# dylanpeifer/deepgroebner

Measured on AMD Instinct MI355X. Metric: env steps/sec (polynomial additions) on 3-20-10-weighted, batch=4096, 1/2/4/8 GPU, higher is better.
Workload: dtype u16 exponents / u32 GF(32003)

## Files before the change

deepgroebner_amd/csrc/bbx_common.h:

```cpp
#pragma once
#include <stdbool.h>
#include <stddef.h>
#include <stdint.h>

#define BBX_P 32003u
#define BBX_POLICY_MAX_ROWS 2048
#define BBX_MAXVARS 8
#ifdef __HIPCC__
#define BBX_HD __host__ __device__
#else
#define BBX_HD
#endif

enum {
  BBX_ST_OK = 0,
  BBX_ST_G_FULL = 1,
  BBX_ST_P_FULL = 2,
  BBX_ST_ARENA_FULL = 3,
  BBX_ST_POLY_TOO_LONG = 4,
  BBX_ST_DEG_OVERFLOW = 5,
  BBX_ST_STARVED = 6,
  BBX_ST_BAD_ACTION = 7,
  BBX_ST_RUNAWAY = 9,
  BBX_ST_GEN_FAIL = 10,
// ... 204 lines not shown
  bool dev = false;
  int at = 0;
  auto uniform = [&](uint32_t scaling, uint32_t past, uint32_t magic) {
    uint32_t ret = acc.raw(at++) - 1u;
    if (ret >= past) { dev = true; ret = 0; }
    return bbx_gen_div(ret, scaling, magic);
  };
  auto degree = [&]() {
    const uint32_t r1 = acc.raw(at), r2 = acc.raw(at + 1);
    at += 2;
    const double pr = bbx_gen_canonical(r1, r2);
    int d = 0;
    for (int i = 0; i < ncp; i++) d += acc.cp(i) < pr ? 1 : 0;
    return d;
  };
  r.c = (flags & 2u) ? BBX_P - 1u : 1u + uniform(67104u, 2147462208u, 64004u);
  int d1 = 0, d2 = 0;
  if (ncp != 0) {
    d1 = degree();
    d2 = (flags & 1u) ? d1 : degree();
  }
  const BbxGenRow row1 = acc.row(d1), row2 = acc.row(d2);
  const uint32_t j1 = row1.off + uniform(row1.scaling, row1.past, row1.magic);
  const uint32_t j2 = row2.off + uniform(row2.scaling, row2.past, row2.magic);
  uint32_t m1[2], m2[2];
  acc.mono(j1, m1); acc.mono(j2, m2);
  const uint64_t k1 = (((uint64_t)m1[1] << 32) | m1[0]) ^ 0x0000FFFFFFFFFFFFull;
  const uint64_t k2 = (((uint64_t)m2[1] << 32) | m2[0]) ^ 0x0000FFFFFFFFFFFFull;
  const bool second = k2 > k1;
  r.lead[0] = second ? m2[0] : m1[0]; r.lead[1] = second ? m2[1] : m1[1];
  r.tail[0] = second ? m1[0] : m2[0]; r.tail[1] = second ? m1[1] : m2[1];
  r.deviated = dev || k1 == k2;
  return r;
}
#endif

static inline BBX_HD uint32_t bbx_coef_mulmod(uint32_t a, uint32_t b) {
  const uint32_t x = a * b;
  const uint32_t q = (uint32_t)(((uint64_t)x * 1099408559ull) >> 45);
  return x - q * BBX_P;
}
static inline BBX_HD uint32_t bbx_ginfo_hot(uint32_t rec_x, uint32_t inv) {
  const uint32_t mt = bbx_coef_mulmod(rec_x >> 16, inv);
  return mt | ((mt ? BBX_P - mt : 0u) << 16);
}
static inline BBX_HD uint32_t bbx_ginfo_record(uint32_t hot_x, uint32_t kept) { (void)hot_x; return kept; }

#define BBX_PEEL_NO_KEY 0xFFFFFFFFu
static inline BBX_HD uint32_t bbx_peel_key(uint32_t deg, uint32_t index) { return (deg << 8) | index; }
static inline BBX_HD uint32_t bbx_peel_key_deg(uint32_t key) { return key >> 8; }
static inline BBX_HD int bbx_peel_key_lane(uint32_t key) { return (int)(key & 63u); }
static inline BBX_HD int bbx_peel_key_bank(uint32_t key) { return (int)((key >> 6) & 3u); }

static inline BBX_HD uint64_t bbx_mix64(uint64_t idx, uint32_t word) {
  uint64_t z = ((idx << 32) | (uint64_t)word) + 0x9E3779B97F4A7C15ull;
  z = (z ^ (z >> 30)) * 0xBF58476D1CE4E5B9ull;
  z = (z ^ (z >> 27)) * 0x94D049BB133111EBull;
  return z ^ (z >> 31);
}
static inline BBX_HD uint32_t bbx_agent_hash32(uint32_t seed, uint32_t t) {
  return (uint32_t)(bbx_mix64((uint64_t)seed, t) >> 32);
}
static inline BBX_HD uint32_t bbx_agent_action32(uint32_t seed, uint32_t t, uint32_t rows) {
  return (uint32_t)(((uint64_t)bbx_agent_hash32(seed, t) * rows) >> 32);
}
```

deepgroebner_amd/csrc/bbx_fast.h:

```cpp
#pragma once

typedef Mono<2> M2;
template <int NBK> struct FLay {
  static constexpr int G = 64 * NBK, P = 2 * G, OVF = G > 128 ? G - 128 : 0;
  static constexpr int OFF_LM = 0, OFF_TM = 8 * G, OFF_GI = 16 * G, OFF_PR = 24 * G, OFF_SX = 24 * G + 4 * P, OFF_GC = OFF_SX + 2 * OVF;
  static constexpr int BYTES = OFF_GC + 4 * G;
};
constexpr int FNBK_WIDE = 4, FNBK_POL = 2;
static_assert(FLay<FNBK_WIDE>::BYTES == 9472 && FLay<FNBK_POL>::BYTES == 4608, "FLay: bytes per environment (DESIGN.md 4.1, LDS budget)");
static_assert(FLay<FNBK_WIDE>::OFF_GC % 4 == 0 && FLay<FNBK_WIDE>::BYTES % 16 == 0 && FLay<FNBK_POL>::BYTES % 16 == 0, "FLay: alignment of gc[] and of the next wave's region");
static_assert(16 * FLay<FNBK_WIDE>::BYTES == 151552 && 16 * FLay<FNBK_WIDE>::BYTES <= 160 * 1024, "16 environments per CU no longer fit its LDS");
static_assert(16 * (FLay<FNBK_POL>::BYTES + 4 * FLay<FNBK_POL>::P) + 66576 == 156688 && 156688 <= 160 * 1024, "policy2<128,128>: 16 environments per CU no longer fit its LDS");
constexpr uint32_t FSENT = 0xFFFFFFFFu;

struct BbxFastParams {
  char* recs; const uint32_t* qwords; const int32_t* qtail; const uint16_t* inv_table;
  const int32_t* actions; double* rewards; uint8_t* dones; int32_t* rows; int32_t* obs; BbxTraceRec* trace;
  uint32_t rec_bytes, hbmG;
  uint32_t q_env_stride, q_slot_words, q_nslots, q_fixed;
  int32_t B, nsteps, obs_rows, trace_stride, k, nvars, lim_G, lim_P;
  int32_t agent, auto_reset, set_budget, pass, obs_every_step, obs_fill, rewards_mode;
  int32_t* lite;
  int32_t done_seq;
  const uint32_t* gen;
// ... 142 lines not shown
  int budget_in = uni(ghdr->budget), rollout_pos = uni(ghdr->rollout_pos), done_in = uni(ghdr->done_last);
  if (status == BBX_ST_STARVED || status == BBX_ST_SPILL || status == BBX_ST_TIMESLICE) status = BBX_ST_OK;
  if (p.set_budget) { budget_in = bbx_st_capacity(status) ? budget_in + p.nsteps : p.nsteps; rollout_pos = 0; done_in = 0; }
  if (p.sess_target) budget_in = p.sess_target - uni(ghdr->sess_done);
  const uint32_t t_begin = PERSIST ? (uint32_t)__builtin_amdgcn_s_memrealtime() : 0u;
  int mb_action = -1;
  bool mb_pending = false;
  int pol_t0 = 0;
  if (POL > 0 && PERSIST) { int vz_; asm volatile("v_mov_b32 %0, 0" : "=v"(vz_)); pol_t0 = vz_ + (t_agent - (p.set_budget ? 0 : uni(ghdr->sess_done))); }
  if (p.pass == 1 && !(status == BBX_ST_OK && (need_reset || (budget_in > 0 && nP > 0)))) return;
  if constexpr (PERSIST) {
    if (p.sess_target && !p.set_budget && !p.mbox && uni(ghdr->status) == BBX_ST_OK && !need_reset && budget_in <= 0 &&
        nG <= (p.lim_G < FG ? p.lim_G : FG) && nP <= (p.lim_P < FP ? p.lim_P : FP)) {
      const unsigned long long w = __hip_atomic_load(p.ctl, __ATOMIC_RELAXED, __HIP_MEMORY_SCOPE_AGENT);
      if (uni((int)(uint32_t)w) <= uni(ghdr->sess_done) && (uni((int)(uint32_t)(w >> 32)) & 1)) {
        if (lane == 0) {
          const int done_last = done_in ? 1 : 0;
          const int trunc_all = ghdr->obs_trunc | ((POL == 0 && p.obs && nP > p.obs_rows) ? 1 : 0);
          ghdr->arena_used = 0; ghdr->steps_done = 0; ghdr->budget = budget_in; ghdr->done_last = done_last; ghdr->obs_trunc = trunc_all;
          if (p.dones) p.dones[env] = (uint8_t)bbx_done_flag(done_last, nP, 0);
          if (p.rows) p.rows[env] = nP;
          if (p.lite) {
            int32_t* lw = p.lite + 4 * (size_t)env;
            const int word0 = bbx_lite_word0(BBX_ST_OK, trunc_all, p.done_seq);
            if (p.done_seq) {
              lw[1] = q_head; lw[2] = budget_in; lw[3] = nP;
              __threadfence_system();
              __hip_atomic_store(lw, word0, __ATOMIC_RELEASE, __HIP_MEMORY_SCOPE_SYSTEM);
            } else *(int4*)lw = make_int4(word0, q_head, budget_in, nP);
          }
        }
        return;
      }
    }
  }
  int t_stop = t_agent + budget_in, t_event = t_agent;

#define F_HBM_PTRS(PP) \
  const uint32_t HG = (PP)->hbmG; char* grec_ = (PP)->recs + (size_t)env * (PP)->rec_bytes; \
  M2* g_lm = (M2*)(grec_ + 128);            M2* g_tm = (M2*)(grec_ + 128 + 8 * HG); \
  M2* g_slm = (M2*)(grec_ + 128 + 16 * HG); M2* g_stm = (M2*)(grec_ + 128 + 24 * HG); \
  uint2* g_gi = (uint2*)(grec_ + 128 + 40 * HG); uint2* g_si = (uint2*)(grec_ + 128 + 48 * HG); \
  uint32_t* g_pr = (uint32_t*)(grec_ + 128 + 56 * HG);
  char* lbase = smem + wave_in_block * (FLDS_BYTES + (POL > 0 ? 4 * FP : 0));
  M2* lm = (M2*)(lbase + FOFF_LM); M2* tm = (M2*)(lbase + FOFF_TM);
  uint2* gi = (uint2*)(lbase + FOFF_GI); uint32_t* pairs = (uint32_t*)(lbase + FOFF_PR);
  uint32_t* gc = (uint32_t*)(lbase + LY::OFF_GC);
  const int limG = p.lim_G < FG ? p.lim_G : FG, limP = p.lim_P < FP ? p.lim_P : FP;

  uint16_t* sx = (uint16_t*)(lbase + LY::OFF_SX);
  FastState S;
  auto clear_reducers = [&]() { f_banks<FRB>([&](auto b_) { constexpr int b = decltype(b_)::value; S.slm[b].w[0] = S.slm[b].w[1] = FSENT; }); };
  clear_reducers();
  f_banks<FRB>([&](auto b_) { constexpr int b = decltype(b_)::value; S.stm[b] = m_zero<2>(); S.sin[b] = make_uint2(0, 0); });
  bool staged_in = false;
  const bool idle0 = !PERSIST && !need_reset && nP == 0;
  if (status == BBX_ST_OK && !idle0) {
    if (nG > limG || nP > limP) status = BBX_ST_SPILL;
    else {
      F_HBM_PTRS(&p)
      f_banks<NBK>([&](auto b_) {
        constexpr int b = decltype(b_)::value;
        const int i = lane + 64 * b;
        if (i < nG) {
          if constexpr (b < FRB) { S.slm[b] = g_slm[i]; S.stm[b] = g_stm[i]; S.sin[b] = g_si[i]; }
          else sx[i - 64 * FRB] = (uint16_t)(g_si[i].y >> 16);
          const uint2 rg = g_gi[i];
          lm[i] = g_lm[i]; tm[i] = g_tm[i]; gc[i] = rg.x; gi[i] = make_uint2(bbx_ginfo_hot(rg.x, rg.y & 0xffffu), rg.y);
        }
      });
      for (int i = lane; i < nP; i += WAVE) pairs[i] = g_pr[i];
      staged_in = true;
      wave_sync();
    }
  }
  f_loads_landed();
  uint32_t PA = pairs[lane];

  uint32_t hv = bbx_agent_hash32(agent_seed, (uint32_t)((t_agent & ~63) + lane));
  int vzero; asm volatile("v_mov_b32 %0, 0" : "=v"(vzero));
  int adds = vzero, episodes = vzero, zero_red = vzero;
  int trace_pos = rollout_pos;
  long long bytes_total = 0;
  int last_nred = vzero - 1;
  int obs_rows_max = vzero;
  int t_done = vzero + (done_in ? t_agent : t_agent - 1);
  const int t_entry = vzero + t_agent;
  int t_ep0 = 0, t_lim = 0;
  if constexpr (!NOLIM) {
    t_ep0 = vzero + (t_agent - uni(ghdr->episode_steps));
    t_lim = uni(bbx_episode_tlim(t_agent - uni(ghdr->episode_steps), t_agent, p.episode_limit));
  }
  const bool tracing = TRACE && p.trace != nullptr;
  const int n = HL ? 3 : p.nvars, kk = HL ? 2 : p.k;
  const int agent = HL ? BBX_AGENT_HASH : p.agent;
  const bool auto_reset = HL ? true : p.auto_reset != 0;
  const bool obs_fill = HL ? false : p.obs_fill != 0;
  int filled_to = (!HL && p.obs_fill == 2 && p.rows) ? uni(p.rows[env]) : 0x7fffffff;
  const bool obs_step = HL ? true : (POL > 0 ? false : (p.obs_every_step && p.obs));
  const int per_row = 2 * kk;
  const int obs_row_bytes = 4 * per_row * n;
  const int o_rl = lane / per_row, o_slot = lane - o_rl * per_row;
  const int rows_per_sweep = per_row <= WAVE ? WAVE / per_row : 0;

  struct __attribute__((aligned(4))) ObsI3 { int32_t a, b, c; };
  const bool obs32 = HL ? true : (n == 3 && kk == 2 && p.obs != nullptr);
  const int o3_row = lane >> 2, o3_hi = (lane >> 1) & 1;
  const char* o3_mono = lbase + ((lane & 1) ? FOFF_TM : FOFF_LM);
  int32_t* const o3_base = obs32 ? p.obs + (size_t)env * p.obs_rows * 12 : nullptr;
  typedef int32_t ObsV3 __attribute__((ext_vector_type(3)));
  size_t o3_toff = 0;
  auto note_rows = [&]() { obs_rows_max = obs_rows_max > nP ? obs_rows_max : nP; };
  auto write_obs32 = [&]() {
    const int rows = nP < p.obs_rows ? nP : p.obs_rows;
    int32_t* ob = o3_base + o3_toff;
    asm volatile("" : "+s"(ob));
    const __amdgpu_buffer_rsrc_t rs = __builtin_amdgcn_make_buffer_rsrc((void*)ob, 0, rows * 48, 0x00020000);
    int r0 = 0;
// ... 118 lines not shown
            if (valid[b]) { eq[b] = ballot64(f_u64(L[b]) == ls) & valid[b]; dv[b] = ballot64(m_divides(Ls, L[b])); }
            bad |= eq[b] & cp[b];
          }
        });
        if (bad == 0) f_banks<BK>([&](auto b_) { constexpr int b = decltype(b_)::value; if (BK == 1 || sb == b) emit[b] |= 1ull << s; });
        f_banks<BK>([&](auto b_) { constexpr int b = decltype(b_)::value; cand[b] &= ~dv[b]; });
      }
    }
    auto stays = [&](uint32_t pr, const M2& li, const M2& lj, int k) {
      const uint32_t a0 = pk_max(li.w[0], lj.w[0]), a1 = pk_max(li.w[1], lj.w[1]);
      const uint32_t b0 = pk_max(li.w[0], f.w[0]), b1 = pk_max(li.w[1], f.w[1]);
      const uint32_t c0 = pk_max(lj.w[0], f.w[0]), c1 = pk_max(lj.w[1], f.w[1]);
      const bool fdiv = (pk_subsat(f.w[0], a0) | (pk_subsat(f.w[1], a1) & 0xffffu)) == 0;
      const bool eqi = ((a0 ^ b0) | ((a1 ^ b1) & 0xffffu)) == 0;
      const bool eqj = ((a0 ^ c0) | ((a1 ^ c1) & 0xffffu)) == 0;
      return (k < nP_old) & (k != skip) & !(fdiv & !eqi & !eqj);
    };
    const bool keep_first = stays(pr_first, li_first, lj_first, lane);
    const uint64_t mask_first = ballot64(keep_first);
    if (keep_first) pairs[f_prefix(mask_first)] = pr_first;
    int w = __popcll(mask_first);
    for (int base = WAVE; base < nP_old; base += WAVE) {
      const int k = base + lane;
      const uint32_t pr = k < nP_old ? pairs[k] : 0u;
      const bool keep = stays(pr, lm[pr & 0xffffu], lm[pr >> 16], k);
      const uint64_t mask = ballot64(keep);
      if (keep) pairs[w + f_prefix(mask)] = pr;
      w += __popcll(mask);
    }
    nP = w;
    f_banks<BK>([&](auto b_) {
      constexpr int b = decltype(b_)::value;
      if (b == 0 || emit[b]) {
        if (f_lane_in(emit[b])) pairs[nP + f_prefix(emit[b])] = (uint32_t)(lane + 64 * b) | ((uint32_t)g << 16);
        nP += __popcll(emit[b]);
      }
    });
    {
      constexpr int RB = BK < FRB ? BK : FRB;
      int pos = __popcll(ballot64(!m_gt(S.slm[0], f)));
      f_banks<RB>([&](auto b_) {
        constexpr int b = decltype(b_)::value;
        if constexpr (b > 0) if (g >= 64 * b) pos += __popcll(ballot64(!m_gt(S.slm[b], f)));
      });
      const int novf = (OVF && BK > FRB && g > 64 * FRB) ? g - 64 * FRB : 0;
      if (OVF && BK > FRB) for (int k0 = 0; k0 < novf; k0 += WAVE) {
        const int k = k0 + lane;
        const bool le = k < novf && !m_gt(lm[sx[k < novf ? k : 0]], f);
        pos += __popcll(ballot64(le));
      }
      const uint32_t inv = (uint32_t)uni((int)inv_raw);
      const uint32_t rec_x = t0.c | (t1.c << 16), hot_x = bbx_ginfo_hot(rec_x, inv);
      if (lane == 0) { lm[g] = f; tm[g] = tail; gi[g] = make_uint2(hot_x, inv | ((uint32_t)sugar << 16)); gc[g] = rec_x; }
      const uint2 ns = make_uint2(t1.c | (hot_x & 0xffff0000u), (uint32_t)sugar | ((uint32_t)g << 16));
      int ovq = -1; uint32_t ovg = 0;
      if (OVF && BK > FRB && g >= 64 * FRB) {
        if (pos >= 64 * FRB) { ovq = pos - 64 * FRB; ovg = (uint32_t)g; }
        else { ovq = 0; ovg = f_readlane(S.sin[FRB - 1].y, 63) >> 16; }
      }
      if (!(OVF && BK > FRB) || pos < 64 * FRB) {
        const int pb = RB == 1 ? 0 : pos >> 6, q = RB == 1 ? pos : pos & 63;
        uint32_t c0 = 0, c1 = 0, c2 = 0, c3 = 0, c4 = 0, c5 = 0;
        const uint32_t nv[6] = {f.w[0], f.w[1], tail.w[0], tail.w[1], ns.x, ns.y};
        f_banks<RB>([&](auto b_) {
          constexpr int b = decltype(b_)::value;
          if (RB == 1 || pb == b) {
            if constexpr (b + 1 < RB) {
              c0 = f_readlane(S.slm[b].w[0], 63); c1 = f_readlane(S.slm[b].w[1], 63); c2 = f_readlane(S.stm[b].w[0], 63);
              c3 = f_readlane(S.stm[b].w[1], 63); c4 = f_readlane(S.sin[b].x, 63); c5 = f_readlane(S.sin[b].y, 63);
            }
            f_insert6(S.slm[b].w[0], S.slm[b].w[1], S.stm[b].w[0], S.stm[b].w[1], S.sin[b].x, S.sin[b].y, nv, q);
          } else if (b > 0 && pb < b && g >= 64 * b) {
            c0 = f_shift_in(S.slm[b].w[0], c0, lane); c1 = f_shift_in(S.slm[b].w[1], c1, lane);
            c2 = f_shift_in(S.stm[b].w[0], c2, lane); c3 = f_shift_in(S.stm[b].w[1], c3, lane);
            c4 = f_shift_in(S.sin[b].x, c4, lane); c5 = f_shift_in(S.sin[b].y, c5, lane);
          }
        });
      }
      if (OVF && BK > FRB && ovq >= 0) {
        for (int k0 = ((novf - 1 - ovq) / WAVE) * WAVE; k0 >= 0; k0 -= WAVE) {
          const int k = ovq + k0 + lane;
          uint16_t v = 0;
          if (k < novf) v = sx[k];
          wave_sync();
          if (k < novf) sx[k + 1] = v;
          wave_sync();
        }
        if (lane == 0) sx[ovq] = (uint16_t)ovg;
      }
    }
    nG = g + 1;
    wave_sync();
    PA = pairs[lane];
  };

  auto install_ideal = [&](int n, bool in_order) {
    int ln = lane; asm volatile("" : "+v"(ln));
    const bool mine = ln < n;
    const M2 L = lm[ln];
    {
      const M2 T = tm[ln];
      const uint32_t cx = gi[ln].x, sugar = m_deg(L);
      if (mine) gc[ln] = 1u | (cx << 16);
      const int rk = in_order ? ln : gen_sorted_rank<2>(L, n);
      const int to = 4 * (mine ? rk : ln);
      auto put = [&](uint32_t v) { return (uint32_t)__builtin_amdgcn_ds_permute(to, (int)v); };
      S.slm[0].w[0] = put(mine ? L.w[0] : FSENT); S.slm[0].w[1] = put(mine ? L.w[1] : FSENT);
      S.stm[0].w[0] = put(T.w[0]); S.stm[0].w[1] = put(T.w[1]);
      S.sin[0].x = put(cx); S.sin[0].y = put(sugar | ((uint32_t)ln << 16));
    }
    int j = 0;
#pragma unroll
    for (int t = 1; t <= 10; t++) j += ln >= t * (t - 1) / 2 ? 1 : 0;
    const int i = ln - ((j * (j - 1)) >> 1);
    auto get = [&](int from, const M2& v) { M2 r; r.w[0] = (uint32_t)__builtin_amdgcn_ds_bpermute(4 * from, (int)v.w[0]);
                                            r.w[1] = (uint32_t)__builtin_amdgcn_ds_bpermute(4 * from, (int)v.w[1]); return r; };
    const M2 Li = get(i, L), Lj = get(j, L), Lij = m_lcm(Li, Lj);
    bool keep = ln < ((n * (n - 1)) >> 1);
    for (int k = 0; k < n; k++) {
      const M2 Lk = f_readlane(L, k);
      const M2 Lkj = m_lcm(Lk, Lj);
      const bool eq = m_eq(Lkj, Lij);
      const bool not_new = (m_divides(Lkj, Lij) && !eq) || (eq && (k < i || m_coprime(Lk, Lj)));
      const bool dropped = m_divides(Lk, Lij) && !eq && !m_eq(Lij, m_lcm(Li, Lk));
      keep = keep && !(k < j ? not_new : (k > j && dropped));
    }
    const uint64_t kept = ballot64(keep);
    if (keep) pairs[f_prefix(kept)] = (uint32_t)i | ((uint32_t)j << 16);
    nG = n; nP = __popcll(kept);
    wave_sync();
    PA = pairs[lane];
  };

#ifndef BBX_PRIO_SHIFT
#define BBX_PRIO_SHIFT 6
#endif
  static_assert(BBX_PRIO_SHIFT == 6, "one test serves the hash refill, the priority rotation and the time slice");
  for (;;) {
    nP = uni(nP);
    if (__builtin_expect(t_agent == t_event, 0)) {
      if (status != BBX_ST_OK) break;
      if (need_reset) {
        bool ok = true;
        const FColdParams cq = f_cold_params();
        const uint32_t* gtab = cq->gen;
        if (gtab) {
          const int npoly = (int)ldc(gtab + 2), ncp = (int)ldc(gtab + 4);
          const uint32_t gflags = ldc(gtab + 3);
          const GenLanes GL = gen_lanes(gtab);
          uint32_t x = (uint32_t)uni((int)gen_state);
          FSTAMP(0);
          for (;;) {
            const uint32_t x_start = x;
            nG = 0; nP = 0;
            clear_reducers();
            const bool sorted = cq->sort_input != 0;
            const bool one_pass = npoly <= 11 && limG >= npoly && limP >= npoly + ((npoly * (npoly - 1)) >> 1);
            M2 tabL = m_zero<2>(), tabT = m_zero<2>(); uint32_t tabC = 0; int rank = 0;
            const bool batch = one_pass && gen_ideal_lanes(x, gtab, GL, gflags, ncp, npoly, tabL, tabT, tabC);
            if (sorted) {
              for (int fidx = 0; fidx < npoly && ok && !batch; fidx++) {
                M2 lead, tail; uint32_t c;
// ... 227 lines not shown
    }
    else if (!HL && agent >= BBX_AGENT_NORMAL && agent <= BBX_AGENT_SPICE) action = uni(f_select_ordered(pairs, lm, gi, nP, agent));
    else {
      uint32_t best = 0xFFFFFFFFu;
      for (int r = lane; r < nP; r += WAVE) {
        const uint32_t pr = pairs[r];
        const uint32_t key = (m_deg(m_lcm(lm[pr & 0xffffu], lm[pr >> 16])) << 16) | (uint32_t)r;
        best = key < best ? key : best;
      }
      action = (int)(f_wave_min(best) & 0xffffu);
    }
    if (!(HL || agent == BBX_AGENT_HASH) && (action < 0 || action >= nP)) { status = BBX_ST_BAD_ACTION; break; }
    uint32_t pr = f_readlane(PA, action & 63);
    if (action >= 64) pr = (uint32_t)uni((int)pairs[action]);
    const int gi_ = pr & 0xffffu, gj_ = pr >> 16;
    FSTAMP(1);
    BTerm<2> h0, h1;
    int hsug, bytes;
    {
      const M2 lmi = lm[gi_], lmj = lm[gj_];
      uint2 ii = gi[gi_], ij = gi[gj_];
      const M2 tmi = tm[gi_], tmj = tm[gj_];
      asm volatile("" : "+v"(ii.x), "+v"(ii.y), "+v"(ij.x), "+v"(ij.y));
      const M2 gamma = m_lcm(lmi, lmj);
      const M2 si = m_div(gamma, lmi), sj = m_div(gamma, lmj);
      BTerm<2> a, b;
      a.c = ii.x & 0xffffu;   a.m = m_mul(tmi, si);
      b.c = ij.x >> 16;       b.m = m_mul(tmj, sj);
      const int sgi = (int)(ii.y >> 16) + (int)m_deg(si), sgj = (int)(ij.y >> 16) + (int)m_deg(sj);
      hsug = uni(sgi > sgj ? sgi : sgj);
      if constexpr (ACCT) merge2<2>(a, b, h0, h1); else { h0 = a; h1 = b; }
      bytes = ACCT ? 12 * ((a.c ? 2 : 1) + (b.c ? 2 : 1) + (h0.c ? 1 : 0) + (h1.c ? 1 : 0)) : 0;
    }

    FSTAMP(2);
    uint32_t h0c = (uint32_t)uni((int)h0.c), h0a = (uint32_t)uni((int)h0.m.w[0]), h0b = (uint32_t)uni((int)h0.m.w[1]);
    uint32_t h1c = (uint32_t)uni((int)h1.c), h1a = (uint32_t)uni((int)h1.m.w[0]), h1b = (uint32_t)uni((int)h1.m.w[1]);
    uint32_t r0c = 0, r0a = 0, r0b = 0, r1c = 0, r1a = 0, r1b = 0;
    int nred = 0, rsug = 0;
    const int ngu = uni(nG);
    auto round_cpp = [&](auto regs) {
      const int hn = h1c ? 2 : 1;
      M2 hm; hm.w[0] = h0a; hm.w[1] = h0b;
      int found = -1;
      uint32_t nb0 = 0, nb1 = 0, sxw = 0;
      int fs = 0;
      if constexpr (decltype(regs)::value) f_banks<FRB>([&](auto b_) {
        constexpr int b = decltype(b_)::value;
        if (found < 0 && (b == 0 || ngu > 64 * b)) {
          const uint64_t mb = ballot64(m_divides(S.slm[b], hm));
          if (mb) {
            const int l = __builtin_ctzll(mb);
            found = 64 * b + l;
            const uint32_t q1 = h0b - S.slm[b].w[1];
            nb0 = f_readlane(S.stm[b].w[0] + (h0a - S.slm[b].w[0]), l); nb1 = f_readlane(S.stm[b].w[1] + q1, l);
            sxw = f_readlane(S.sin[b].x, l); fs = (int)f_readlane((S.sin[b].y & 0xffffu) + (q1 >> 16), l);
          }
        }
      });
      if (OVF && found < 0 && ngu > 64 * FRB) {
        const int novf = ngu - 64 * FRB;
        for (int k0 = 0; k0 < novf && found < 0; k0 += WAVE) {
          const int k = k0 + lane;
          const int gk = k < novf ? (int)sx[k] : 0;
          const M2 fl = lm[gk];
          const uint64_t mb = ballot64(k < novf && m_divides(fl, hm));
          if (mb) {
            const int l = __builtin_ctzll(mb);
            found = 64 * FRB + k0 + l;
            const int gs = (int)f_readlane((uint32_t)gk, l);
            const M2 fm = f_readlane(fl, l), ft = tm[gs];
            const uint2 info = gi[gs];
            const uint32_t tc = gc[gs] >> 16, q1 = h0b - fm.w[1];
            nb0 = (uint32_t)uni((int)(ft.w[0] + (h0a - fm.w[0]))); nb1 = (uint32_t)uni((int)(ft.w[1] + q1));
            sxw = (uint32_t)uni((int)(tc | (info.x & 0xffff0000u)));
            fs = uni((int)((info.y >> 16) + (q1 >> 16)));
          }
        }
      }
      if (found >= 0) {
        const uint32_t tcg = sxw & 0xffffu, kg = sxw >> 16;
        hsug = fs > hsug ? fs : hsug;
        if (hsug > 65535) return;
        h0c = mulmod(h0c, kg);
        h0a = nb0; h0b = nb1;
        if (ACCT) bytes += 8 * (found + 1) + 12 * (tcg ? 2 : 1) + 12 * hn;
        if (h0c == 0) { h0c = h1c; h0a = h1a; h0b = h1b; h1c = 0; }
        else if (h1c != 0) {
          const uint64_t kx = (((uint64_t)h1b << 32) | h1a) ^ 0x0000FFFFFFFFFFFFull;
          const uint64_t ky = (((uint64_t)h0b << 32) | h0a) ^ 0x0000FFFFFFFFFFFFull;
          if (kx > ky) {
            const uint32_t tc_ = h0c, ta_ = h0a, tb_ = h0b;
            h0c = h1c; h0a = h1a; h0b = h1b; h1c = tc_; h1a = ta_; h1b = tb_;
          } else if (kx == ky) { h0c = addmod(h0c, h1c); h1c = 0; }
        }
        if (ACCT) bytes += 12 * ((h0c ? 1 : 0) + (h1c ? 1 : 0));
        nred++;
      } else {
        if (ACCT) bytes += 8 * ngu + 12 * (2 * hn - 1);
        if (r0c == 0) { r0c = h0c; r0a = h0a; r0b = h0b; } else { r1c = h0c; r1a = h0a; r1b = h0b; }
        const int d = (int)(h0b >> 16);
        rsug = d > rsug ? d : rsug;
        h0c = h1c; h0a = h1a; h0b = h1b; h1c = 0;
      }
    };
    if constexpr (!ACCT) {
      const int ng_s = ngu;
      uint32_t nred_u = 0, rsug_u = 0, hsug_u = (uint32_t)hsug;
      uint32_t sl, sf, sx_, sxx, sq;
      uint32_t t0, t1, t2;
#define FA_SCAN(P) \
        "v_pk_sub_u16 %[t0], %[" #P "lm0], %[h0a] clamp\n\t" \
        "v_pk_sub_u16 %[t1], %[" #P "lm1], %[h0b] clamp\n\t" \
        "s_nop 0\n\t" \
        "v_or_b32 %[t0], %[t0], %[t1]\n\t" \
        "v_cmp_eq_u32 vcc, 0, %[t0]\n\t" \
        "v_sub_u32 %[t1], %[h0b], %[" #P "lm1]\n\t" \
        "v_sub_u32 %[t0], %[h0a], %[" #P "lm0]\n\t" \
        "v_add_u32 %[t2], %[t1], %[" #P "tm1]\n\t" \
        "v_add_u32 %[t0], %[t0], %[" #P "tm0]\n\t" \
        "v_lshrrev_b32 %[t1], 16, %[t1]\n\t" \
        "v_add_u32 %[t1], %[t1], %[" #P "sug]\n\t"
#define FA_PICK(P) \
        "s_ff1_i32_b64 %[sl], vcc\n\t" \
        "v_readlane_b32 %[sf], %[t1], %[sl]\n\t" \
        "v_readlane_b32 %[sx], %[" #P "inx], %[sl]\n\t" \
        "s_max_i32 %[hsug], %[hsug], %[sf]\n\t" \
        "s_cmp_gt_i32 %[hsug], 0xffff\n\t" \
        "s_cbranch_scc1 L_done_%=\n\t" \
        "v_readlane_b32 %[h0a], %[t0], %[sl]\n\t" \
        "v_readlane_b32 %[h0b], %[t2], %[sl]\n\t"
#define FA_TRY(P, NGMIN, NEXT) \
        "L_try" #P "_%=:\n\t" \
        "s_cmp_lt_i32 %[ng], " #NGMIN "\n\t" \
        "s_cbranch_scc1 L_tm_%=\n\t" \
        FA_SCAN(P) \
        "s_cbranch_vccz " NEXT "_%=\n\t" \
        FA_PICK(P) \
        "s_branch L_red_%=\n\t"
#define FA_ORDER(N, LAST) \
        "s_cmp_eq_u32 %[h0c], 0\n\t" \
        "s_cbranch_scc1 L_shift" N "_%=\n\t" \
        "s_cmp_eq_u32 %[h1c], 0\n\t" \
        "s_cbranch_scc1 L_top_%=\n\t" \
        "s_xor_b32 %[sxx], %[h1b], 0xffff\n\t"            \
        "s_xor_b32 %[sq], %[h0b], 0xffff\n\t" \
        "s_cmp_lt_u32 %[sxx], %[sq]\n\t" \
        "s_cbranch_scc1 L_top_%=\n\t"                      \
        "s_cmp_eq_u32 %[sxx], %[sq]\n\t" \
        "s_cbranch_scc0 L_swap" N "_%=\n\t" \
        "s_cmp_lt_u32 %[h1a], %[h0a]\n\t" \
        "s_cbranch_scc1 L_swap" N "_%=\n\t" \
        "s_cmp_eq_u32 %[h1a], %[h0a]\n\t" \
        "s_cbranch_scc0 L_top_%=\n\t" \
        "s_add_u32 %[sxx], %[h0c], %[h1c]\n\t"             \
        "s_add_u32 %[sq], %[sxx], 0xffff82fd\n\t" \
        "s_min_u32 %[h0c], %[sxx], %[sq]\n\t" \
        "s_mov_b32 %[h1c], 0\n\t" \
        "s_branch L_top_%=\n\t" \
        "L_swap" N "_%=:\n\t"                                   \
        "s_mov_b32 %[sxx], %[h0c]\n\t" "s_mov_b32 %[h0c], %[h1c]\n\t" "s_mov_b32 %[h1c], %[sxx]\n\t" \
        "s_mov_b32 %[sxx], %[h0a]\n\t" "s_mov_b32 %[h0a], %[h1a]\n\t" "s_mov_b32 %[h1a], %[sxx]\n\t" \
        "s_mov_b32 %[sxx], %[h0b]\n\t" "s_mov_b32 %[h0b], %[h1b]\n\t" "s_mov_b32 %[h1b], %[sxx]\n\t" \
        "s_branch L_top_%=\n\t" \
        "L_shift" N "_%=:\n\t"                                  \
        "s_mov_b32 %[h0c], %[h1c]\n\t" "s_mov_b32 %[h0a], %[h1a]\n\t" "s_mov_b32 %[h0b], %[h1b]\n\t" "s_mov_b32 %[h1c], 0\n\t" \
        LAST
#define FA_HEAD(NEXT) \
        FA_ORDER("0", "") \
        "L_top_%=:\n\t" \
        "s_cmp_eq_u32 %[h0c], 0\n\t" \
        "s_cbranch_scc1 L_done_%=\n\t" \
        FA_SCAN(a) \
        "s_cbranch_vccz " NEXT "_%=\n\t" \
        FA_PICK(a) \
        "L_red_%=:\n\t"                                    \
        "s_lshr_b32 %[sq], %[sx], 16\n\t" \
        "s_mul_i32 %[sxx], %[h0c], %[sq]\n\t" \
        "s_mul_hi_u32 %[sq], %[sxx], 0x4187a4af\n\t" \
        "s_lshr_b32 %[sq], %[sq], 13\n\t" \
        "s_mul_i32 %[sq], %[sq], 0x7d03\n\t" \
        "s_sub_u32 %[h0c], %[sxx], %[sq]\n\t" \
        "s_add_u32 %[nred], %[nred], 1\n\t" \
        FA_ORDER("", "s_branch L_top_%=\n\t")
#define FA_TAIL \
        "L_tm_%=:\n\t"                                     \
        "s_cmp_eq_u32 %[r0c], 0\n\t" \
        "s_cbranch_scc0 L_tm1_%=\n\t" \
        "s_mov_b32 %[r0c], %[h0c]\n\t" "s_mov_b32 %[r0a], %[h0a]\n\t" "s_mov_b32 %[r0b], %[h0b]\n\t" \
        "s_branch L_tm2_%=\n\t" \
        "L_tm1_%=:\n\t" \
        "s_mov_b32 %[r1c], %[h0c]\n\t" "s_mov_b32 %[r1a], %[h0a]\n\t" "s_mov_b32 %[r1b], %[h0b]\n\t" \
        "L_tm2_%=:\n\t" \
        "s_lshr_b32 %[sxx], %[h0b], 16\n\t" \
        "s_max_i32 %[rsug], %[rsug], %[sxx]\n\t" \
        "s_mov_b32 %[h0c], %[h1c]\n\t" "s_mov_b32 %[h0a], %[h1a]\n\t" "s_mov_b32 %[h0b], %[h1b]\n\t" "s_mov_b32 %[h1c], 0\n\t" \
        "s_branch L_top_%=\n\t" \
        "L_done_%=:"
#define FA_OUTS \
          [h0c] "+s"(h0c), [h0a] "+s"(h0a), [h0b] "+s"(h0b), [h1c] "+s"(h1c), [h1a] "+s"(h1a), [h1b] "+s"(h1b), \
          [r0c] "+s"(r0c), [r0a] "=&s"(r0a), [r0b] "=&s"(r0b), [r1c] "+s"(r1c), [r1a] "=&s"(r1a), [r1b] "=&s"(r1b), \
          [nred] "+s"(nred_u), [rsug] "+s"(rsug_u), [hsug] "+s"(hsug_u), \
          [sl] "=&s"(sl), [sf] "=&s"(sf), [sx] "=&s"(sx_), [sxx] "=&s"(sxx), [sq] "=&s"(sq), \
          [t0] "=&v"(t0), [t1] "=&v"(t1), [t2] "=&v"(t2)
#define FA_BANK(P, b) \
          [P##lm0] "v"(S.slm[b].w[0]), [P##lm1] "v"(S.slm[b].w[1]), [P##tm0] "v"(S.stm[b].w[0]), [P##tm1] "v"(S.stm[b].w[1]), \
          [P##inx] "v"(S.sin[b].x), [P##sug] "v"(S.sin[b].y & 0xffffu)
      if constexpr (!OVF) {
        asm volatile(FA_HEAD("L_tryb") FA_TRY(b, 65, "L_tm") FA_TAIL
                     : FA_OUTS : FA_BANK(a, 0), FA_BANK(b, 1), [ng] "s"(ng_s) : "vcc", "scc");
      } else {
        asm volatile(FA_HEAD("L_tryb") FA_TRY(b, 65, "L_ovf")
                     "L_ovf_%=:\n\t"
                     "s_cmp_lt_i32 %[ng], 129\n\t"
                     "s_cbranch_scc1 L_tm_%=\n\t"
                     "s_bitset1_b32 %[nred], 31\n\t"
                     "s_branch L_done_%=\n\t"
                     FA_TAIL
                     : FA_OUTS : FA_BANK(a, 0), FA_BANK(b, 1), [ng] "s"(ng_s) : "vcc", "scc");
      }
#undef FA_SCAN
#undef FA_PICK
#undef FA_TRY
#undef FA_HEAD
#undef FA_ORDER
#undef FA_TAIL
#undef FA_OUTS
#undef FA_BANK
      nred = (int)nred_u; rsug = (int)rsug_u; hsug = (int)hsug_u;
      if (OVF && __builtin_expect(nred < 0, 0)) {
        nred &= 0x7fffffff;
        while (h0c != 0 && hsug <= 65535) round_cpp(std::true_type{});
      }
    } else
    while (h0c != 0 && hsug <= 65535) round_cpp(std::true_type{});
    if (hsug > 65535) { status = BBX_ST_DEG_OVERFLOW; break; }
    rsug = rsug > hsug ? rsug : hsug;
    BTerm<2> r0, r1;
    r0.c = r0c; r0.m.w[0] = r0a; r0.m.w[1] = r0b; r1.c = r1c; r1.m.w[0] = r1a; r1.m.w[1] = r1b;

    FSTAMP(3);
    const int nG_before = nG, nP_before = nP - 1;
    if (uni((int)r0.c) == 0) {
      if (nP <= 64) {
        const uint32_t sh = f_wave_shl(PA);
        const bool moved = lane >= action && lane < nP - 1;
        PA = lane >= action ? sh : PA;
        if (moved) pairs[lane] = PA;
      } else {
        for (int base = action; base < nP - 1; base += WAVE) {
          const int k = base + lane;
          uint32_t v = 0;
          if (k < nP - 1) v = pairs[k + 1];
          wave_sync();
          if (k < nP - 1) pairs[k] = v;
          wave_sync();
        }
        PA = pairs[lane];
      }
      nP -= 1;
// ... 30 lines not shown
          for (int v = 0; v < BBX_MAXVARS; v++) nh += bbx_mix64(2 + v, v < 3 ? m_exp(r0.m, v) : 0u);
          if (r1.c) {
            nh += bbx_mix64(10, r1.c);
            for (int v = 0; v < BBX_MAXVARS; v++) nh += bbx_mix64(11 + v, v < 3 ? m_exp(r1.m, v) : 0u);
          }
        }
        nh = wave_sum64(nh);
      }
      if (lane == 0) {
        BbxTraceRec& tr = p.trace[(size_t)env * p.trace_stride + trace_pos];
        tr.action = action; tr.nP = nP; tr.nG = nG; tr.done = done ? 1 : 0;
        tr.reward = p.rewards_mode == BBX_REW_ADDITIONS ? (-1.0 - (double)nred) : -1.0;
        tr.obs_hash = oh; tr.pairs_hash = ph; tr.newpoly_hash = nh;
      }
    }
    if constexpr (POL > 0) {
      const FColdPolicy pol = f_cold_policy();
      if (pol->post_obs && p.obs) { write_obs32(); note_rows(); }
      if (lane == 0) {
        const size_t tb = (size_t)pol_tt * (size_t)pol->stride_out + (size_t)env;
        if (pol->rewards_t) pol->rewards_t[tb] = p.rewards_mode == BBX_REW_ADDITIONS ? (-1.0 - (double)nred) : -1.0;
        if (pol->dones_t) pol->dones_t[tb] = done ? 1 : 0;
        if (pol->post_obs && pol->rows_t) pol->rows_t[env] = nP;
      }
    }
    if constexpr (PERSIST && POL == 0 && !HL) {
      if (f_cold_params()->mbox) { mb_pending = true; t_event = t_agent; }
    }
    if (TRACE) trace_pos++;
    if constexpr (NOLIM) {
    if (done) { episodes++; t_done = vzero + t_agent; t_event = t_agent; if (auto_reset) need_reset = 1; }
    } else if (done) {
      const int lim = f_cold_params()->episode_limit, esteps = t_agent - uni(t_ep0);
      const int end = bbx_episode_end(nP, esteps, lim);
      if (bbx_episode_counted(end, esteps, lim, auto_reset ? 1 : 0)) { episodes++; if (end == 2) count_truncation((BbxHdr*)(f_cold_params()->recs + (size_t)env * f_cold_params()->rec_bytes)); }
      t_done = vzero + t_agent; t_event = t_agent;
      if (auto_reset) need_reset = 1; else t_lim = uni(bbx_episode_tlim(uni(t_ep0), t_agent, lim));
    }
    FSTAMP(5);
  }
  const FColdParams cz = f_cold_params();
  if (PROF && cz->prof && lane == 0) for (int i = 0; i < 8; i++) cz->prof[(size_t)env * 8 + i] = prof_sum[i];

  const bool handoff = status == BBX_ST_SPILL;
  if (handoff && lane == 0 && cz->ctl_stats) atomicAdd((unsigned long long*)cz->ctl_stats + 1, 1ull);
  if (POL == 0 && p.obs && status == BBX_ST_OK) { if (obs32) write_obs32(); else write_obs(true, false); note_rows(); }
  if (staged_in) {
    wave_sync();
    F_HBM_PTRS(cz)
    f_banks<NBK>([&](auto b_) {
      constexpr int b = decltype(b_)::value;
      const int i = lane + 64 * b;
      if (i < nG) {
        if constexpr (b < FRB) { g_slm[i] = S.slm[b]; g_stm[i] = S.stm[b]; g_si[i] = S.sin[b]; }
        else {
          const int gk = sx[i - 64 * FRB];
          const uint2 info = gi[gk];
          g_slm[i] = lm[gk]; g_stm[i] = tm[gk];
          g_si[i] = make_uint2((gc[gk] >> 16) | (info.x & 0xffff0000u), (info.y >> 16) | ((uint32_t)gk << 16));
        }
        const uint2 wi = gi[i];
        g_lm[i] = lm[i]; g_tm[i] = tm[i]; g_gi[i] = make_uint2(bbx_ginfo_record(wi.x, gc[i]), wi.y);
      }
    });
    for (int i = lane; i < nP; i += WAVE) g_pr[i] = pairs[i];
  }
  if (lane == 0) {
    BbxHdr* h = (BbxHdr*)(cz->recs + (size_t)env * cz->rec_bytes);
    const int budget = t_stop - t_agent, done_last = t_done == t_agent ? 1 : 0;
    const int obs_trunc = obs_rows_max > cz->obs_rows ? 1 : 0;
    const int budget0 = cz->sess_target ? cz->sess_target - h->sess_done
                                        : (cz->set_budget ? (bbx_st_capacity(status) ? h->budget + cz->nsteps : cz->nsteps) : h->budget);
    const int steps_done = PERSIST ? t_agent - h->t : budget0 - budget;
    if (PERSIST) {
      h->sess_done = (cz->set_budget ? 0 : h->sess_done) + steps_done;
      if (!cz->set_budget && steps_done > 0 && cz->ctl_stats) atomicAdd((unsigned long long*)cz->ctl_stats, (unsigned long long)steps_done);
    } else if (cz->sess_target) h->sess_done = cz->sess_target - budget;
    rollout_pos = (cz->set_budget ? 0 : h->rollout_pos) + steps_done;
    h->nG = nG; h->nP = nP; h->arena_used = 0; h->status = status; h->need_reset = need_reset;
    h->q_head = q_head; h->t = t_agent; h->total_steps += steps_done; h->total_additions += adds;
    h->gen_rng = gen_state;
    if (!HL) h->std_rng = std_rng;
    if (VAL) { h->vret = vret; h->vdisc = vdisc; if (cz->values) cz->values[env] = vret; }
    h->episodes += episodes; h->zero_reductions += zero_red; h->steps_done = steps_done;
    if constexpr (!NOLIM) h->episode_steps = t_agent - t_ep0;
    h->budget = budget; h->rollout_pos = rollout_pos; h->done_last = done_last; h->alg_bytes += bytes_total;
    const int trunc_all = (cz->set_budget ? 0 : h->obs_trunc) | obs_trunc;
    h->obs_trunc = trunc_all;
    if (!handoff) {
      double* rw = cz->rewards; uint8_t* dn = cz->dones; int32_t* rws = cz->rows;
      if (rw && (steps_done > 0 || (cz->pass == 0 && !cz->sess_target)))
        rw[env] = last_nred < 0 ? 0.0 : (cz->rewards_mode == BBX_REW_ADDITIONS ? (-1.0 - (double)last_nred) : -1.0);
      if (dn) dn[env] = (uint8_t)((done_last || (nP == 0 && !need_reset)) ? 1 : 0);
      if (rws) rws[env] = nP;
    }
    if (cz->lite) {
      const int seq = (PERSIST && cz->mbox) ? bbx_lite_seq_of(h->sess_done) : cz->done_seq;
      int32_t* lw = cz->lite + 4 * (size_t)env;
      const int word0 = bbx_lite_word0(status, trunc_all, seq);
      if (seq) {
        lw[1] = q_head; lw[2] = budget; lw[3] = nP;
        __threadfence_system();
        __hip_atomic_store(lw, word0, __ATOMIC_RELEASE, __HIP_MEMORY_SCOPE_SYSTEM);
        if (PERSIST && cz->mbox) __hip_atomic_store(lw + 2, budget | BBX_LITE_GONE, __ATOMIC_RELEASE, __HIP_MEMORY_SCOPE_SYSTEM);
      } else *(int4*)lw = make_int4(word0, q_head, budget, nP);
    }
  }
// ... 54 lines not shown
```

Baseline: 2.224 billion.

## Store reducer tails as deltas from leads to shorten the reduction scan

Reducer tail monomials and sugar are now kept in registers as differences from the reducer's lead monomial, so a reduction step becomes one scalar add after reading the matching lane. The vector subtract/add/shift work in the per-bank scan is removed and replaced by readlanes plus scalar arithmetic, which also frees one VGPR temporary. Values are converted back to absolute form when written to HBM and converted on load. This relies on wraparound arithmetic of packed u16 exponents and sugar staying consistent across every place the reducer registers are written, including the sentinel initialisation and the permute-based rebuild.

```diff
diff --git a/deepgroebner_amd/csrc/bbx_common.h b/deepgroebner_amd/csrc/bbx_common.h
--- a/deepgroebner_amd/csrc/bbx_common.h
+++ b/deepgroebner_amd/csrc/bbx_common.h
@@ -280,6 +280,15 @@
 static inline BBX_HD int bbx_peel_key_lane(uint32_t key) { return (int)(key & 63u); }
 static inline BBX_HD int bbx_peel_key_bank(uint32_t key) { return (int)((key >> 6) & 3u); }
 
+static inline BBX_HD uint32_t bbx_red_delta(uint32_t lm_w, uint32_t tm_w) { return tm_w - lm_w; }
+static inline BBX_HD uint32_t bbx_red_tail(uint32_t lm_w, uint32_t d_w) { return d_w + lm_w; }
+static inline BBX_HD uint32_t bbx_red_esugar(uint32_t sugar, uint32_t lm_w1) { return (sugar - (lm_w1 >> 16)) & 0xffffu; }
+static inline BBX_HD uint32_t bbx_red_sugar(uint32_t e, uint32_t lm_w1) { return (e + (lm_w1 >> 16)) & 0xffffu; }
+static inline BBX_HD uint32_t bbx_red_info_hot(uint32_t y, uint32_t lm_w1) { return (y & 0xffff0000u) | bbx_red_esugar(y & 0xffffu, lm_w1); }
+static inline BBX_HD uint32_t bbx_red_info_record(uint32_t y, uint32_t lm_w1) { return (y & 0xffff0000u) | bbx_red_sugar(y & 0xffffu, lm_w1); }
+static inline BBX_HD uint32_t bbx_red_step(uint32_t h_w, uint32_t d_w) { return h_w + d_w; }
+static inline BBX_HD uint32_t bbx_red_step_sugar(uint32_t e, uint32_t h_w1) { return e + (h_w1 >> 16); }
+
 static inline BBX_HD uint64_t bbx_mix64(uint64_t idx, uint32_t word) {
   uint64_t z = ((idx << 32) | (uint64_t)word) + 0x9E3779B97F4A7C15ull;
   z = (z ^ (z >> 30)) * 0xBF58476D1CE4E5B9ull;
diff --git a/deepgroebner_amd/csrc/bbx_fast.h b/deepgroebner_amd/csrc/bbx_fast.h
--- a/deepgroebner_amd/csrc/bbx_fast.h
+++ b/deepgroebner_amd/csrc/bbx_fast.h
@@ -218,7 +218,10 @@
   FastState S;
   auto clear_reducers = [&]() { f_banks<FRB>([&](auto b_) { constexpr int b = decltype(b_)::value; S.slm[b].w[0] = S.slm[b].w[1] = FSENT; }); };
   clear_reducers();
-  f_banks<FRB>([&](auto b_) { constexpr int b = decltype(b_)::value; S.stm[b] = m_zero<2>(); S.sin[b] = make_uint2(0, 0); });
+  f_banks<FRB>([&](auto b_) {
+    constexpr int b = decltype(b_)::value;
+    S.stm[b].w[0] = S.stm[b].w[1] = bbx_red_delta(FSENT, 0u); S.sin[b] = make_uint2(0, bbx_red_info_hot(0u, FSENT));
+  });
   bool staged_in = false;
   const bool idle0 = !PERSIST && !need_reset && nP == 0;
   if (status == BBX_ST_OK && !idle0) {
@@ -229,7 +232,11 @@
         constexpr int b = decltype(b_)::value;
         const int i = lane + 64 * b;
         if (i < nG) {
-          if constexpr (b < FRB) { S.slm[b] = g_slm[i]; S.stm[b] = g_stm[i]; S.sin[b] = g_si[i]; }
+          if constexpr (b < FRB) {
+            const M2 rl = g_slm[i], rt = g_stm[i]; const uint2 ri = g_si[i];
+            S.slm[b] = rl; S.stm[b].w[0] = bbx_red_delta(rl.w[0], rt.w[0]); S.stm[b].w[1] = bbx_red_delta(rl.w[1], rt.w[1]);
+            S.sin[b] = make_uint2(ri.x, bbx_red_info_hot(ri.y, rl.w[1]));
+          }
           else sx[i - 64 * FRB] = (uint16_t)(g_si[i].y >> 16);
           const uint2 rg = g_gi[i];
           lm[i] = g_lm[i]; tm[i] = g_tm[i]; gc[i] = rg.x; gi[i] = make_uint2(bbx_ginfo_hot(rg.x, rg.y & 0xffffu), rg.y);
@@ -454,7 +461,7 @@
       const uint32_t inv = (uint32_t)uni((int)inv_raw);
       const uint32_t rec_x = t0.c | (t1.c << 16), hot_x = bbx_ginfo_hot(rec_x, inv);
       if (lane == 0) { lm[g] = f; tm[g] = tail; gi[g] = make_uint2(hot_x, inv | ((uint32_t)sugar << 16)); gc[g] = rec_x; }
-      const uint2 ns = make_uint2(t1.c | (hot_x & 0xffff0000u), (uint32_t)sugar | ((uint32_t)g << 16));
+      const uint2 ns = make_uint2(t1.c | (hot_x & 0xffff0000u), bbx_red_esugar((uint32_t)sugar, f.w[1]) | ((uint32_t)g << 16));
       int ovq = -1; uint32_t ovg = 0;
       if (OVF && BK > FRB && g >= 64 * FRB) {
         if (pos >= 64 * FRB) { ovq = pos - 64 * FRB; ovg = (uint32_t)g; }
@@ -463,7 +470,7 @@
       if (!(OVF && BK > FRB) || pos < 64 * FRB) {
         const int pb = RB == 1 ? 0 : pos >> 6, q = RB == 1 ? pos : pos & 63;
         uint32_t c0 = 0, c1 = 0, c2 = 0, c3 = 0, c4 = 0, c5 = 0;
-        const uint32_t nv[6] = {f.w[0], f.w[1], tail.w[0], tail.w[1], ns.x, ns.y};
+        const uint32_t nv[6] = {f.w[0], f.w[1], bbx_red_delta(f.w[0], tail.w[0]), bbx_red_delta(f.w[1], tail.w[1]), ns.x, ns.y};
         f_banks<RB>([&](auto b_) {
           constexpr int b = decltype(b_)::value;
           if (RB == 1 || pb == b) {
@@ -508,8 +515,8 @@
       const int to = 4 * (mine ? rk : ln);
       auto put = [&](uint32_t v) { return (uint32_t)__builtin_amdgcn_ds_permute(to, (int)v); };
       S.slm[0].w[0] = put(mine ? L.w[0] : FSENT); S.slm[0].w[1] = put(mine ? L.w[1] : FSENT);
-      S.stm[0].w[0] = put(T.w[0]); S.stm[0].w[1] = put(T.w[1]);
-      S.sin[0].x = put(cx); S.sin[0].y = put(sugar | ((uint32_t)ln << 16));
+      S.stm[0].w[0] = bbx_red_delta(S.slm[0].w[0], put(T.w[0])); S.stm[0].w[1] = bbx_red_delta(S.slm[0].w[1], put(T.w[1]));
+      S.sin[0].x = put(cx); S.sin[0].y = bbx_red_info_hot(put(sugar | ((uint32_t)ln << 16)), S.slm[0].w[1]);
     }
     int j = 0;
 #pragma unroll
@@ -843,9 +850,9 @@
           if (mb) {
             const int l = __builtin_ctzll(mb);
             found = 64 * b + l;
-            const uint32_t q1 = h0b - S.slm[b].w[1];
-            nb0 = f_readlane(S.stm[b].w[0] + (h0a - S.slm[b].w[0]), l); nb1 = f_readlane(S.stm[b].w[1] + q1, l);
-            sxw = f_readlane(S.sin[b].x, l); fs = (int)f_readlane((S.sin[b].y & 0xffffu) + (q1 >> 16), l);
+            fs = (int)bbx_red_step_sugar(f_readlane(S.sin[b].y, l) & 0xffffu, h0b);
+            nb0 = bbx_red_step(h0a, f_readlane(S.stm[b].w[0], l)); nb1 = bbx_red_step(h0b, f_readlane(S.stm[b].w[1], l));
+            sxw = f_readlane(S.sin[b].x, l);
           }
         }
       });
@@ -899,28 +906,27 @@
       const int ng_s = ngu;
       uint32_t nred_u = 0, rsug_u = 0, hsug_u = (uint32_t)hsug;
       uint32_t sl, sf, sx_, sxx, sq;
-      uint32_t t0, t1, t2;
+      uint32_t t0, t1;
 #define FA_SCAN(P) \
         "v_pk_sub_u16 %[t0], %[" #P "lm0], %[h0a] clamp\n\t" \
         "v_pk_sub_u16 %[t1], %[" #P "lm1], %[h0b] clamp\n\t" \
         "s_nop 0\n\t" \
         "v_or_b32 %[t0], %[t0], %[t1]\n\t" \
-        "v_cmp_eq_u32 vcc, 0, %[t0]\n\t" \
-        "v_sub_u32 %[t1], %[h0b], %[" #P "lm1]\n\t" \
-        "v_sub_u32 %[t0], %[h0a], %[" #P "lm0]\n\t" \
-        "v_add_u32 %[t2], %[t1], %[" #P "tm1]\n\t" \
-        "v_add_u32 %[t0], %[t0], %[" #P "tm0]\n\t" \
-        "v_lshrrev_b32 %[t1], 16, %[t1]\n\t" \
-        "v_add_u32 %[t1], %[t1], %[" #P "sug]\n\t"
+        "v_cmp_eq_u32 vcc, 0, %[t0]\n\t"
 #define FA_PICK(P) \
         "s_ff1_i32_b64 %[sl], vcc\n\t" \
-        "v_readlane_b32 %[sf], %[t1], %[sl]\n\t" \
+        "v_readlane_b32 %[sf], %[" #P "sug], %[sl]\n\t" \
         "v_readlane_b32 %[sx], %[" #P "inx], %[sl]\n\t" \
+        "v_readlane_b32 %[sq], %[" #P "tm0], %[sl]\n\t" \
+        "v_readlane_b32 %[sxx], %[" #P "tm1], %[sl]\n\t"       \
+        "s_lshr_b32 %[sl], %[h0b], 16\n\t" \
+        "s_and_b32 %[sf], %[sf], 0xffff\n\t" \
+        "s_add_u32 %[sf], %[sf], %[sl]\n\t" \
         "s_max_i32 %[hsug], %[hsug], %[sf]\n\t" \
         "s_cmp_gt_i32 %[hsug], 0xffff\n\t" \
         "s_cbranch_scc1 L_done_%=\n\t" \
-        "v_readlane_b32 %[h0a], %[t0], %[sl]\n\t" \
-        "v_readlane_b32 %[h0b], %[t2], %[sl]\n\t"
+        "s_add_u32 %[h0a], %[h0a], %[sq]\n\t" \
+        "s_add_u32 %[h0b], %[h0b], %[sxx]\n\t"
 #define FA_TRY(P, NGMIN, NEXT) \
         "L_try" #P "_%=:\n\t" \
         "s_cmp_lt_i32 %[ng], " #NGMIN "\n\t" \
@@ -993,10 +999,10 @@
           [r0c] "+s"(r0c), [r0a] "=&s"(r0a), [r0b] "=&s"(r0b), [r1c] "+s"(r1c), [r1a] "=&s"(r1a), [r1b] "=&s"(r1b), \
           [nred] "+s"(nred_u), [rsug] "+s"(rsug_u), [hsug] "+s"(hsug_u), \
           [sl] "=&s"(sl), [sf] "=&s"(sf), [sx] "=&s"(sx_), [sxx] "=&s"(sxx), [sq] "=&s"(sq), \
-          [t0] "=&v"(t0), [t1] "=&v"(t1), [t2] "=&v"(t2)
+          [t0] "=&v"(t0), [t1] "=&v"(t1)
 #define FA_BANK(P, b) \
           [P##lm0] "v"(S.slm[b].w[0]), [P##lm1] "v"(S.slm[b].w[1]), [P##tm0] "v"(S.stm[b].w[0]), [P##tm1] "v"(S.stm[b].w[1]), \
-          [P##inx] "v"(S.sin[b].x), [P##sug] "v"(S.sin[b].y & 0xffffu)
+          [P##inx] "v"(S.sin[b].x), [P##sug] "v"(S.sin[b].y)
       if constexpr (!OVF) {
         asm volatile(FA_HEAD("L_tryb") FA_TRY(b, 65, "L_tm") FA_TAIL
                      : FA_OUTS : FA_BANK(a, 0), FA_BANK(b, 1), [ng] "s"(ng_s) : "vcc", "scc");
@@ -1133,7 +1139,10 @@
       constexpr int b = decltype(b_)::value;
       const int i = lane + 64 * b;
       if (i < nG) {
-        if constexpr (b < FRB) { g_slm[i] = S.slm[b]; g_stm[i] = S.stm[b]; g_si[i] = S.sin[b]; }
+        if constexpr (b < FRB) {
+          M2 rt; rt.w[0] = bbx_red_tail(S.slm[b].w[0], S.stm[b].w[0]); rt.w[1] = bbx_red_tail(S.slm[b].w[1], S.stm[b].w[1]);
+          g_slm[i] = S.slm[b]; g_stm[i] = rt; g_si[i] = make_uint2(S.sin[b].x, bbx_red_info_record(S.sin[b].y, S.slm[b].w[1]));
+        }
         else {
           const int gk = sx[i - 64 * FRB];
           const uint2 info = gi[gk];
```

Result: no change. 2.223 billion (-0.0%).
